# opendedup/sdfs

Hardware: AMD Instinct MI355X
Metric: device-resident GiB/s CDC+fingerprint, 4 KiB-mean chunks, 1/2/4/8 MI355X (higher is better)
Workload: dtype u8; 1 GPU; 64 streams x 64 MiB per GPU, CHUNK_LENGTH 262144 B (16384 buffers, 4.00 GiB per GPU), fresh CDC state per buffer; chunks_per_gpu_step=1059575, streams_in_flight=2, exchange=none (N=1), parallelism=dp1 (streams sharded per GPU)

## Files before the change

### sdfs_amd/csrc/cdc_device.h

```cpp
#pragma once

#include "cdc_internal.h"

namespace sdfs {

__device__ __forceinline__ uint32_t xor3(uint32_t a, uint32_t b, uint32_t c) {
    return __builtin_amdgcn_bitop3_b32(a, b, c, 0x96);
}
__device__ __forceinline__ uint32_t maj3(uint32_t a, uint32_t b, uint32_t c) {
    return __builtin_amdgcn_bitop3_b32(a, b, c, 0xE8);
}
__device__ __forceinline__ uint32_t bitop3_and_or(uint32_t a, uint32_t b, uint32_t c) {
    return __builtin_amdgcn_bitop3_b32(a, b, c, 0xEA);
}

constexpr int kAblMirror = 64;
constexpr int kAblSgprPred = 256;
constexpr int kAblFullBlocks = 512;

constexpr int kAblSdwa = 1024;
constexpr int kAblSdwaPop = 2048;
constexpr int kAblMinGroup = 4096;
constexpr int kAblMinGroup8 = 8192;
constexpr int kAblPopSwap = 16384;
constexpr int kAblPopMux = 32768;

template <int B>
__device__ __forceinline__ void sdwa_byte_to_b1(uint32_t& d, uint32_t src) {
    static_assert(B >= 0 && B < 4, "byte select");
    if constexpr (B == 0)
        asm("v_mov_b32_sdwa %0, %1 dst_sel:BYTE_1 dst_unused:UNUSED_PRESERVE src0_sel:BYTE_0" : "+v"(d) : "v"(src));
    else if constexpr (B == 1)
        asm("v_mov_b32_sdwa %0, %1 dst_sel:BYTE_1 dst_unused:UNUSED_PRESERVE src0_sel:BYTE_1" : "+v"(d) : "v"(src));
    else if constexpr (B == 2)
        asm("v_mov_b32_sdwa %0, %1 dst_sel:BYTE_1 dst_unused:UNUSED_PRESERVE src0_sel:BYTE_2" : "+v"(d) : "v"(src));
    else
        asm("v_mov_b32_sdwa %0, %1 dst_sel:BYTE_1 dst_unused:UNUSED_PRESERVE src0_sel:BYTE_3" : "+v"(d) : "v"(src));
}

template <int P, int Q, int ABL = 0>
__device__ __forceinline__ void roll_step(uint32_t& lo, uint32_t& hi, uint32_t dw, uint32_t odw, uint32_t& c8,
                                          uint32_t& push_base, uint32_t jshift, const uint8_t* tab) {
    if constexpr ((ABL & kAblMirror) != 0) {
        uint32_t pa, qa;
        if constexpr ((ABL & kAblSdwa) != 0) {
            asm("v_lshrrev_b32_sdwa %0, %2, %1 dst_sel:BYTE_1 dst_unused:UNUSED_PRESERVE src0_sel:DWORD src1_sel:DWORD"
                : "+v"(push_base)
                : "v"(lo), "s"(jshift));
            pa = push_base;
        } else {
            pa = bitop3_and_or(lo >> (jshift - 8), 0xFF00u, push_base);
        }
        if constexpr ((ABL & kAblSdwaPop) != 0 && (ABL & kAblPopMux) != 0 && Q == 2) {
            qa = __builtin_amdgcn_bitop3_b32(odw, 0xFF00u, c8, 0xE2);
        } else if constexpr ((ABL & kAblSdwaPop) != 0) {
            sdwa_byte_to_b1<3 - Q>(c8, odw);
            qa = c8;
        } else {
            qa = Q == 2 ? bitop3_and_or(odw, 0xFF00u, c8)
                        : __builtin_amdgcn_perm(odw, c8, 0x0C0C0000u | ((4u + 3 - Q) << 8));
        }
        const uint2 pv = (ABL & 2) ? make_uint2(pa, pa >> 3) : *reinterpret_cast<const uint2*>(tab + pa);
        const uint2 qv = (ABL & 1) ? make_uint2(qa, qa >> 3) : *reinterpret_cast<const uint2*>(tab + qa);
        const uint32_t nlo = __builtin_amdgcn_alignbit(hi, lo, 8);
        const uint32_t nhi = __builtin_amdgcn_perm(hi, dw, 0x00070605u | ((3u - P) << 24));
        if constexpr ((ABL & kAblPopSwap) != 0) {
            lo = xor3(nlo, pv.x, qv.y);
            hi = xor3(nhi, pv.y, qv.x);
        } else {
            lo = xor3(nlo, pv.x, qv.x);
            hi = xor3(nhi, pv.y, qv.y);
        }
        return;
    }
    const uint32_t pa = bitop3_and_or(hi >> (jshift - 8), 0xFF00u, push_base);
    const uint32_t qa = __builtin_amdgcn_perm(odw, c8, 0x0C0C0000u | ((4u + Q) << 8));
    const uint2 pv = (ABL & 2) ? make_uint2(pa, pa >> 3) : *reinterpret_cast<const uint2*>(tab + pa);
    const uint2 qv = (ABL & 1) ? make_uint2(qa, qa >> 3) : *reinterpret_cast<const uint2*>(tab + qa);
    const uint32_t nhi = __builtin_amdgcn_alignbit(hi, lo, 24);
    const uint32_t nlo = __builtin_amdgcn_perm(lo, dw, 0x06050400u | P);
    lo = xor3(nlo, pv.x, qv.x);
    hi = xor3(nhi, pv.y, qv.y);
}

template <int P, bool M = false>
__device__ __forceinline__ void push_step(uint32_t& lo, uint32_t& hi, uint32_t dw, uint32_t push_base,
                                          uint32_t jshift, const uint8_t* tab) {
    if constexpr (M) {
        const uint2 pv = *reinterpret_cast<const uint2*>(tab + bitop3_and_or(lo >> (jshift - 8), 0xFF00u, push_base));
        const uint32_t nlo = __builtin_amdgcn_alignbit(hi, lo, 8);
        const uint32_t nhi = __builtin_amdgcn_perm(hi, dw, 0x00070605u | ((3u - P) << 24));
        lo = nlo ^ pv.x;
        hi = nhi ^ pv.y;
        return;
    }
    const uint2 pv = *reinterpret_cast<const uint2*>(tab + bitop3_and_or(hi >> (jshift - 8), 0xFF00u, push_base));
    const uint32_t nhi = __builtin_amdgcn_alignbit(hi, lo, 24);
    const uint32_t nlo = __builtin_amdgcn_perm(lo, dw, 0x06050400u | P);
    lo = nlo ^ pv.x;
    hi = nhi ^ pv.y;
}

template <int PK>
__device__ __forceinline__ void cand_shift(uint32_t& bits, uint32_t lo, uint32_t hi, const ScanArgs& a) {
    if constexpr (PK == 3) {
        const uint32_t flo = __builtin_bitreverse32(lo), fhi = __builtin_bitreverse32(hi);
        const double f = __builtin_fma((double)fhi, 4294967296.0, (double)flo);
        const double q = __builtin_floor(f * a.div_inv);
        const double r = __builtin_fma(-q, a.div_d, f);
        const uint32_t h = (r == a.rem_d) | (r + a.div_d == a.rem_d) | (r - a.div_d == a.rem_d);
        asm("v_lshl_or_b32 %0, %0, 1, %1" : "+v"(bits) : "v"(h));
    } else if constexpr (PK == 2) {
        asm("v_cmp_gt_u32 vcc, %2, %1\n\t"
            "v_addc_co_u32 %0, vcc, %0, %0, vcc"
            : "+v"(bits)
            : "v"(lo), "s"(a.thr)
            : "vcc");
    } else if constexpr (PK == 1) {
        uint32_t t, t2;
        asm("v_and_b32 %1, %4, %3\n\t"
            "v_xor_b32 %1, %5, %1\n\t"
            "v_and_b32 %2, %7, %6\n\t"
            "v_xor_b32 %2, %8, %2\n\t"
            "v_or_b32 %1, %1, %2\n\t"
            "v_cmp_eq_u32 vcc, 0, %1\n\t"
            "v_addc_co_u32 %0, vcc, %0, %0, vcc"
            : "+v"(bits), "=&v"(t), "=&v"(t2)
            : "v"(lo), "s"(a.mask_lo), "s"(a.val_lo), "v"(hi), "s"(a.mask_hi), "s"(a.val_hi)
            : "vcc");
    } else {
        uint32_t t;
        asm("v_and_b32 %1, %3, %2\n\t"
            "v_cmp_eq_u32 vcc, %4, %1\n\t"
            "v_addc_co_u32 %0, vcc, %0, %0, vcc"
            : "+v"(bits), "=&v"(t)
            : "v"(lo), "s"(a.mask_lo), "s"(a.val_lo)
            : "vcc");
    }
}

template <int W, int PK, int O, int ABL, int BLKW>
__device__ __forceinline__ void byte_step(uint32_t& lo, uint32_t& hi, uint32_t& bits, const uint32_t (&cur)[BLKW],
                                          const uint32_t (&prev)[16], uint32_t& c8, uint32_t& push_base,
                                          const uint8_t* tab, const ScanArgs& a, uint64_t (&gm)[8], uint32_t (&hv)[8]) {
    constexpr int OLD = O - W;
    constexpr int OI = OLD >= 0 ? OLD : OLD + 64;
    const uint32_t odw = OLD >= 0 ? cur[OI >> 2] : prev[OI >> 2];
    roll_step<(O & 3), (OI & 3), ABL>(lo, hi, cur[O >> 2], odw, c8, push_base, a.jshift, tab);
    if constexpr ((ABL & 4) != 0 && (ABL & kAblSgprPred) != 0) {
        asm volatile("" ::"v"(hi));
    } else if constexpr (ABL & 4) {
        bits ^= lo;
    } else if constexpr ((ABL & kAblMinGroup) != 0 && (ABL & kAblMirror) != 0 && PK == 2) {
        constexpr int G = (ABL & kAblMinGroup8) != 0 ? 8 : 4;
        hv[O & (G - 1)] = hi;
        if constexpr ((O & (G - 1)) == G - 1) {
            uint32_t m = min(min(hv[0], hv[1]), hv[2]);
            m = min(m, hv[3]);
            if constexpr (G == 8) {
                m = min(min(m, hv[4]), hv[5]);
                m = min(min(m, hv[6]), hv[7]);
            }
            if (__builtin_expect(__any(m < a.thr), 0)) {
#pragma unroll
                for (int p = 0; p < G; p++) cand_shift<2>(bits, hv[p], 0u, a);
            } else {
                bits <<= G;
            }
        }
    } else if constexpr ((ABL & kAblSgprPred) != 0 && (ABL & kAblMirror) != 0 && PK == 2) {
        asm("v_cmp_gt_u32_e64 %0, %1, %2" : "=s"(gm[O & 7]) : "s"(a.thr), "v"(hi));
        if constexpr ((O & 7) == 7) {
            const uint64_t any = (gm[0] | gm[1]) | (gm[2] | gm[3]) | (gm[4] | gm[5]) | (gm[6] | gm[7]);
            if (__builtin_expect(any != 0, 0)) {
#pragma unroll
                for (int p = 0; p < 8; p++) {
                    uint64_t co;
                    asm volatile("v_addc_co_u32_e64 %0, %1, %0, %0, %2" : "+v"(bits), "=s"(co) : "s"(gm[p]));
// ... 448 lines not shown
                atomicOr(a.overflow, 1u);
            }
        }
        carry_rank += (uint32_t)__builtin_popcountll(cut[k]);
        const uint32_t mx = __builtin_amdgcn_readlane(wave_incl_max(end1), 63);
        carry_pos = mx > carry_pos ? mx : carry_pos;
    }
    if (lane == 0 && probe) {
        a.counts[b] = 0;
    } else if (lane == 0) {
        const uint32_t nchunks = cnt + (start < len ? 1u : 0u);
        if (start < len) {
            if (cnt < a.cap) {
                const uint64_t slot = (uint64_t)b * a.cap + cnt;
                a.starts[slot] = start;
                a.clens[slot] = len - start;
                uint32_t bin = sha_blocks(len - start) >> a.bin_shift;
                bin = bin < a.nbins ? bin : a.nbins - 1;
                atomicAdd(&lhist[bin], 1u);
            } else {
                atomicOr(a.overflow, 1u);
            }
        }
        a.counts[b] = nchunks < a.cap ? nchunks : a.cap;
    }
    return true;
}

__device__ __forceinline__ int64_t find_first_sum(const ResolveArgs& a, uint32_t b, uint32_t lo, uint32_t hi,
                                                  uint32_t lane) {
    const uint32_t sl = a.seg_len;
    const uint64_t spb = a.uniform_len / sl;
    const uint64_t word0 = ((uint64_t)b * a.uniform_len) >> 5;
    for (uint32_t s0 = lo / sl; s0 <= hi / sl; s0 += 64) {
        const uint32_t sj = s0 + lane;
        uint32_t best = 0xFFFFFFFFu;
        if (sj <= hi / sl) {
            const uint32_t* ss = a.seg_sum + ((uint64_t)b * spb + sj) * kSegSumWords;
            const uint4 q = *reinterpret_cast<const uint4*>(ss);
            const uint32_t nc = ss[4], ovf = ss[5];
            const uint32_t base = sj * sl;
            const uint32_t qw[4] = {q.x, q.y, q.z, q.w};
#pragma unroll
            for (int j = 0; j < 8; j++) {
                const uint32_t v = (qw[j >> 1] >> (16 * (j & 1))) & 0xFFFFu;
                const uint32_t c = base + v;
                if (v != 0xFFFFu && c >= lo && c <= hi && c < best) best = c;
            }
            if (best == 0xFFFFFFFFu && nc > kSumCands) {
                uint32_t x = base + ovf > lo ? base + ovf : lo;
                const uint32_t seg_hi = base + sl - 1;
                const uint32_t to = seg_hi < hi ? seg_hi : hi;
                while (x <= to) {
                    uint32_t w = a.bitmap[word0 + (x >> 5)] >> (x & 31);
                    const uint32_t span = to - x;
                    if (span < 31) w &= (2u << span) - 1u;
                    if (w) { best = x + __builtin_ctz(w); break; }
                    x = (x | 31u) + 1u;
                }
            }
        }
        const uint64_t m = __ballot(best != 0xFFFFFFFFu);
        if (m) return (int64_t)__builtin_amdgcn_readlane(best, (int)__builtin_ctzll(m));
    }
    return -1;
}

__device__ __forceinline__ void piece_walk_from_summary(const ResolveArgs& a, uint32_t item, uint32_t r0, uint32_t lane,
                                                        const uint32_t (&sm)[4], uint32_t ncand, uint32_t ovf_off,
                                                        uint32_t seg_len, uint64_t word0) {
    const uint32_t len = a.uniform_len;
    const uint32_t r1 = r0 + 64 * seg_len < len ? r0 + 64 * seg_len : len;
    const uint32_t my_base = r0 + lane * seg_len;
    uint32_t q0 = sm[0], q1 = sm[1], q2 = sm[2], q3 = sm[3];
    {
        const uint32_t sh = kSumCands - (ncand < kSumCands ? ncand : kSumCands);
        if (sh & 4) { q3 = q1; q2 = q0; q1 = 0xFFFFFFFFu; q0 = 0xFFFFFFFFu; }
        if (sh & 2) { q3 = q2; q2 = q1; q1 = q0; q0 = 0xFFFFFFFFu; }
        if (sh & 1) {
            q3 = __builtin_amdgcn_alignbit(q3, q2, 16);
            q2 = __builtin_amdgcn_alignbit(q2, q1, 16);
            q1 = __builtin_amdgcn_alignbit(q1, q0, 16);
            q0 = (q0 << 16) | 0xFFFFu;
        }
    }
    auto head_of = [&](uint32_t top) { return (top >> 16) == 0xFFFFu ? 0xFFFFFFFFu : my_base + (top >> 16); };
    uint32_t head = head_of(q3);
    const bool ovf = ncand > kSumCands;
    uint32_t* sp = a.spec_starts + (uint64_t)item * a.spec_cap;
    uint32_t start = r0, cnt = 0;
    while (start < r1) {
        if (lane == 0 && cnt < a.spec_cap) sp[cnt] = start;
        cnt++;
        const uint32_t lo = start + a.first_off;
        const uint32_t forced = start + a.max_len - 1;
        const uint32_t hi = forced < len - 1 ? forced : len - 1;
        const uint32_t hp = hi < r1 - 1 ? hi : r1 - 1;
        int64_t k = -1;
        if (lo <= hp) {
            for (;;) {
                const bool adv = head < lo;
                if (__ballot(adv) == 0) break;
                if (adv) {
                    q3 = __builtin_amdgcn_alignbit(q3, q2, 16);
                    q2 = __builtin_amdgcn_alignbit(q2, q1, 16);
                    q1 = __builtin_amdgcn_alignbit(q1, q0, 16);
                    q0 = (q0 << 16) | 0xFFFFu;
                    head = head_of(q3);
                }
            }
            uint32_t best = head <= hp ? head : 0xFFFFFFFFu;
            if (ovf && head == 0xFFFFFFFFu) {
                uint32_t x = my_base + ovf_off > lo ? my_base + ovf_off : lo;
                const uint32_t seg_hi = my_base + seg_len - 1;
                const uint32_t to = seg_hi < hp ? seg_hi : hp;
                while (x <= to) {
                    uint32_t w = a.bitmap[word0 + (x >> 5)] >> (x & 31);
                    const uint32_t span = to - x;
                    if (span < 31) w &= (2u << span) - 1u;
                    if (w) { best = x + __builtin_ctz(w); break; }
                    x = (x | 31u) + 1u;
                }
            }
            const uint64_t m = __ballot(best != 0xFFFFFFFFu);
            if (m) k = (int64_t)__builtin_amdgcn_readlane(best, (int)__builtin_ctzll(m));
        }
        if (k < 0) {
            if (hi > r1 - 1) break;
            k = (int64_t)hi;
        }
        start = (uint32_t)k + 1;
    }
    if (lane == 0) a.spec_cnt[item] = cnt < a.spec_cap ? cnt : a.spec_cap;
}

template <int C, int NCH, bool PF, int WPS, int ABL = 0, int BLK = 64, int FUSE = 0, int THREADS = kScanThreads,
          bool MIRROR = false>
struct ScanCfg {
    static constexpr bool kMirror = MIRROR;
    static constexpr bool kPopSwap = MIRROR && (ABL & kAblPopSwap) != 0;
    static constexpr int kFuse = NCH == 1 ? FUSE : (FUSE == 2 ? 2 : 0);
    static constexpr int kThreads = THREADS;
    static constexpr int kAbl = ABL;
    static constexpr int kCopies = C;
    static constexpr int kChains = NCH;
    static constexpr bool kPrefetch = PF;
    static constexpr int kWavesPerSimd = WPS;
    static constexpr int kLds = scan_lds_bytes(C);
    static constexpr uint32_t kPushOff = C == 32 ? 0x10000u : 0x80u;
    static constexpr int kBlk = BLK;
    static constexpr bool kListWalk = kFuse == 2 && NCH == 1 && C == 32;
};

template <int W, int PK, class CFG>
__device__ __forceinline__ void scan_iter(const ScanArgs& a, const uint8_t* tab, uint32_t* lhist, uint64_t base,
                                          uint32_t tid, uint32_t bdim, uint64_t total, uint32_t lane, uint32_t c8,
                                          uint32_t push_base, uint32_t& pa_reg, uint32_t& qa_reg,
                                          uint32_t* wlist = nullptr) {
    constexpr int MB =
        (CFG::kMirror ? kAblMirror : 0) | (CFG::kAbl & (kAblSgprPred | kAblSdwa | kAblSdwaPop | kAblMinGroup | kAblMinGroup8 | kAblPopSwap | kAblPopMux));
    constexpr int NCH = CFG::kChains;
    constexpr int BLK = CFG::kBlk;
    constexpr int BLKW = BLK / 4;
    uint64_t start[NCH], end[NCH];
    uint32_t nblk[NCH];
    bool first[NCH];
    uint32_t maxblk = 0;
#pragma unroll
    for (int c = 0; c < NCH; c++) {
        const uint64_t seg = base + (uint64_t)c * bdim + tid;
        start[c] = end[c] = 0;
        nblk[c] = 0;
        first[c] = true;
        if (seg < total) {
            uint64_t bstart, blen, sidx;
            if (a.uniform_len) {
                const uint64_t spb = (a.uniform_len + a.seg_len - 1) / a.seg_len;
                const uint64_t b = seg / spb;
                sidx = seg - b * spb;
                bstart = b * a.uniform_len;
                blen = a.uniform_len;
            } else {
                uint32_t lo_b = 0, hi_b = a.nbuf;
                while (hi_b - lo_b > 1) {
                    const uint32_t mid = (lo_b + hi_b) >> 1;
                    if (a.seg_prefix[mid] <= seg) lo_b = mid; else hi_b = mid;
                }
                sidx = seg - a.seg_prefix[lo_b];
                bstart = a.offs[lo_b];
                blen = a.lens[lo_b];
            }
            start[c] = bstart + sidx * a.seg_len;
            const uint64_t bend = bstart + blen;
            end[c] = start[c] + a.seg_len < bend ? start[c] + a.seg_len : bend;
            nblk[c] = (uint32_t)((end[c] - start[c] + BLK - 1) / BLK);
            first[c] = start[c] == bstart;
        }
        maxblk = nblk[c] > maxblk ? nblk[c] : maxblk;
    }

    uint32_t lo[NCH], hi[NCH];
    uint32_t prev[NCH][16], cur[NCH][BLKW];
    bool cur_full[NCH];
    uint32_t sm[NCH][4];
    uint32_t ncand[NCH];
    uint32_t ovf_off[NCH];
#pragma unroll
    for (int c = 0; c < NCH; c++) {
        sm[c][0] = sm[c][1] = sm[c][2] = sm[c][3] = 0xFFFFFFFFu;
        ncand[c] = 0;
        ovf_off[c] = 0xFFFFFFFFu;
    }
    const bool sparse_bm = CFG::kFuse == 2 && a.fuse_resolve != 0;
#pragma unroll
    for (int c = 0; c < NCH; c++) {
        if (nblk[c] != 0 && !first[c]) {
            load_block<16>(prev[c], a.data, start[c] - 64, start[c]);
            if constexpr (CFG::kMirror)
#pragma unroll
                for (int i = 0; i < 16; i++) prev[c][i] = __builtin_bitreverse32(prev[c][i]);
        } else {
#pragma unroll
            for (int i = 0; i < 16; i++) prev[c][i] = 0;
        }
        lo[c] = hi[c] = 0;
        warm_from<W, 64 - W, CFG::kMirror>(lo[c], hi[c], prev[c], push_base, a.jshift, tab);
        if constexpr (CFG::kPrefetch) {
            const bool act = nblk[c] != 0;
            cur_full[c] = load_block_nb<BLKW>(cur[c], a.data, a.zero_page, act ? start[c] : 0, act ? end[c] : 0);
        }
    }

    for (uint32_t blk = 0; blk < maxblk; blk++) {
        uint32_t nxt[NCH][CFG::kPrefetch ? BLKW : 1];
        bool nxt_full[NCH];
        uint32_t words[NCH][BLK / 32];
        bool split_fast = false;
        if constexpr ((CFG::kAbl & kAblFullBlocks) != 0) {
#pragma unroll
            for (int c = 0; c < NCH; c++) {
                const uint4* p = reinterpret_cast<const uint4*>(a.data + start[c] + (uint64_t)BLK * blk);
#pragma unroll
                for (int i = 0; i < BLKW / 4; i++) {
                    const uint4 v = p[i];
                    cur[c][4 * i] = v.x; cur[c][4 * i + 1] = v.y; cur[c][4 * i + 2] = v.z; cur[c][4 * i + 3] = v.w;
                }
            }
            block_words<W, PK, 0, BLK / 32, NCH, (CFG::kAbl & 7) | MB, BLKW>(words, lo, hi, cur, prev, qa_reg, pa_reg,
                                                                             tab, a);
            split_fast = true;
        } else if constexpr (CFG::kAbl & 16) {
            bool full = true;
#pragma unroll
            for (int c = 0; c < NCH; c++)
                full = full && blk < nblk[c] && start[c] + (uint64_t)BLK * (blk + 1) <= end[c];
            split_fast = __all(full);
            if (split_fast) {
#pragma unroll
                for (int c = 0; c < NCH; c++) {
                    const uint4* p = reinterpret_cast<const uint4*>(a.data + start[c] + (uint64_t)BLK * blk);
#pragma unroll
                    for (int i = 0; i < BLKW / 4; i++) {
                        const uint4 v = p[i];
                        cur[c][4 * i] = v.x; cur[c][4 * i + 1] = v.y; cur[c][4 * i + 2] = v.z; cur[c][4 * i + 3] = v.w;
                    }
                }
                block_words<W, PK, 0, BLK / 32, NCH, (CFG::kAbl & 3) | MB, BLKW>(words, lo, hi, cur, prev, qa_reg, pa_reg,
                                                                                 tab, a);
            }
        }
        if (!split_fast) {
#pragma unroll
        for (int c = 0; c < NCH; c++) {
            if constexpr (CFG::kPrefetch) {
                fix_block<BLKW>(cur[c], cur_full[c], a.data, start[c] + (uint64_t)BLK * blk, end[c]);
                const bool act = blk + 1 < nblk[c];
                nxt_full[c] = load_block_nb<BLKW>(nxt[c], a.data, a.zero_page,
                                                  act ? start[c] + (uint64_t)BLK * (blk + 1) : 0, act ? end[c] : 0);
            } else if constexpr (CFG::kAbl & 8) {
#pragma unroll
                for (int i = 0; i < BLKW; i++) cur[c][i] = prev[c][i & 15] * 0x9E3779B1u + blk;
            } else {
                const bool act = blk < nblk[c];
                load_block<BLKW>(cur[c], a.data, act ? start[c] + (uint64_t)BLK * blk : 0, act ? end[c] : 0);
            }
        }
        block_words<W, PK, 0, BLK / 32, NCH, (CFG::kAbl & 15) | MB, BLKW>(words, lo, hi, cur, prev, qa_reg, pa_reg, tab, a);
        }
        if constexpr (CFG::kFuse == 2) {
#pragma unroll
            for (int c = 0; c < NCH; c++)
#pragma unroll
                for (int w = 0; w < BLK / 32; w++) {
                    uint32_t bits = blk < nblk[c] ? words[c][w] : 0u;
                    while (bits) {
                        const uint32_t off = blk * BLK + 32 * w + __builtin_ctz(bits);
                        bits &= bits - 1;
                        if (start[c] + off < end[c]) sum_push(sm[c], ncand[c], off);
                    }
                }
        }
#pragma unroll
        for (int c = 0; c < NCH; c++) {
            if constexpr (CFG::kFuse == 2)
                if (ncand[c] > kSumCands && ovf_off[c] == 0xFFFFFFFFu) ovf_off[c] = blk * BLK;
            if (blk < nblk[c] && (!sparse_bm || ncand[c] > kSumCands)) {
                const uint64_t pos = start[c] + (uint64_t)BLK * blk;
                uint32_t* bm = a.bitmap + (pos >> 5);
                if (pos + BLK <= end[c]) {
                    if constexpr (BLK >= 128) {
#pragma unroll
                        for (int w = 0; w < BLK / 32; w += 4)
                            *reinterpret_cast<uint4*>(bm + w) =
                                make_uint4(words[c][w], words[c][w + 1], words[c][w + 2], words[c][w + 3]);
                    } else {
                        *reinterpret_cast<uint2*>(bm) = make_uint2(words[c][0], words[c][1]);
                    }
                } else {
#pragma unroll
                    for (int w = 0; w < BLK / 32; w++)
                        if (pos + 32 * w < end[c]) bm[w] = words[c][w];
                }
            }
#pragma unroll
            for (int i = 0; i < 16; i++) prev[c][i] = cur[c][BLKW - 16 + i];
            if constexpr (CFG::kPrefetch) {
#pragma unroll
                for (int i = 0; i < BLKW; i++) cur[c][i] = nxt[c][i];
                cur_full[c] = nxt_full[c];
            }
        }
    }
    if constexpr (CFG::kFuse != 0) {
        if (a.fuse_resolve && a.skip_walk != 1) {
            const uint64_t seg0 = base + (tid & ~63u);
            __builtin_amdgcn_fence(__ATOMIC_RELEASE, "workgroup");
            __builtin_amdgcn_fence(__ATOMIC_ACQUIRE, "workgroup");
            if constexpr (CFG::kFuse == 2) {
                if (a.fuse_resolve == 2) {
                    if constexpr (NCH == 1) {
                        if (base + tid < total) {
                            uint32_t* ss = a.res.seg_sum + (base + tid) * kSegSumWords;
                            *reinterpret_cast<uint4*>(ss) = make_uint4(sm[0][0], sm[0][1], sm[0][2], sm[0][3]);
                            *reinterpret_cast<uint2*>(ss + 4) = make_uint2(ncand[0], ovf_off[0]);
                        }
                        const uint64_t spb = a.uniform_len / a.seg_len;
                        const uint64_t b = seg0 / spb;
                        const uint32_t piece = (uint32_t)((seg0 - b * spb) >> 6);
                        if (seg0 < total)
                            piece_walk_from_summary(a.res, (uint32_t)b * a.res.nsec + piece, piece * 64 * a.seg_len,
                                                    lane, sm[0], ncand[0], ovf_off[0], a.seg_len,
                                                    (b * a.uniform_len) >> 5);
                    }
                } else {
#pragma unroll
                    for (int c = 0; c < NCH; c++) {
                        const uint64_t sc = seg0 + (uint64_t)c * bdim;
                        if (sc < total) {
                            bool done = false;
                            if constexpr (CFG::kListWalk)
                                if (wlist && a.list_walk)
                                    done = resolve_from_list(a.res, (uint32_t)(sc >> 6), lane, sm[c], ncand[c], a.seg_len,
                                                             lhist, wlist, a.skip_walk);
                            if (!done && a.skip_walk > 1) {
                                if (lane == 0) a.res.counts[(uint32_t)(sc >> 6)] = 0;
                            } else if (!done)
                                resolve_from_summary<(CFG::kAbl & 128) == 0>(a.res, (uint32_t)(sc >> 6), lane, sm[c],
                                                                             ncand[c], ovf_off[c], a.seg_len, lhist);
                        }
                    }
                }
            } else {
                if (seg0 < total) resolve_buffer(a.res, (uint32_t)(seg0 >> 6), lane, lhist);
            }
        }
    }
}

template <int W, int PK, class CFG>
__global__ __launch_bounds__(CFG::kThreads, CFG::kWavesPerSimd) void cdc_scan_kernel(ScanArgs a) {
    static_assert(!CFG::kMirror || !CFG::kPrefetch, "mirrored state: no prefetch");
    static_assert(CFG::kMirror || PK < 2, "the one-compare and divisor predicates need the mirrored state");
    constexpr int NCH = CFG::kChains;
    constexpr int C = CFG::kCopies;
    __shared__ __attribute__((aligned(16))) uint8_t tab[CFG::kLds];
    __shared__ uint32_t lhist[CFG::kFuse ? kMaxBins : 1];
    __shared__ uint32_t wlist[CFG::kListWalk ? CFG::kThreads / 64 * kListCap : 1];
    {
        const uint4* src = reinterpret_cast<const uint4*>(a.tab_image);
        uint4* dst = reinterpret_cast<uint4*>(tab);
        for (int i = threadIdx.x; i < CFG::kLds / 16; i += blockDim.x) dst[i] = src[i];
        if constexpr (CFG::kFuse != 0)
            for (uint32_t i = threadIdx.x; i < kMaxBins; i += blockDim.x) lhist[i] = 0;
    }
    __syncthreads();

    const uint32_t lane = threadIdx.x & 63;
    const uint32_t c8 = (lane & (C - 1)) << 3;
    const uint32_t push_base = CFG::kPushOff | c8;
    uint32_t pa_reg = push_base, qa_reg = c8;
    const uint64_t total = a.uniform_len ? a.total_segs : a.seg_prefix[a.nbuf];
    const uint64_t per_iter = (uint64_t)blockDim.x * NCH;

    uint32_t* const wl = CFG::kListWalk ? wlist + (threadIdx.x >> 6) * kListCap : nullptr;
    bool dyn = false;
    if constexpr (NCH == 1) dyn = a.wave_ctr != nullptr;
    const uint32_t items = (uint32_t)((total + 63) >> 6);
    uint64_t sbase = (uint64_t)blockIdx.x * per_iter;
    for (;;) {
        uint64_t base;
        uint32_t tid, bdim;
        if (dyn) {
            uint32_t it = 0;
            if (lane == 0) it = atomicAdd(a.wave_ctr, 1u);
            it = __builtin_amdgcn_readfirstlane(it);
            if (it >= items) break;
            base = (uint64_t)it * 64;
            tid = lane;
            bdim = 64;
        } else {
            if (sbase >= total) break;
            base = sbase;
            tid = threadIdx.x;
            bdim = blockDim.x;
            sbase += (uint64_t)gridDim.x * per_iter;
        }
        scan_iter<W, PK, CFG>(a, tab, lhist, base, tid, bdim, total, lane, c8, push_base, pa_reg, qa_reg, wl);
    }
    if constexpr (CFG::kFuse != 0) {
        if (a.fuse_resolve && a.skip_walk < 2) {
            __syncthreads();
            for (uint32_t i = threadIdx.x; i < a.res.nbins; i += blockDim.x)
                if (lhist[i]) atomicAdd(&a.res.hist[i], lhist[i]);
        }
    }
}

__device__ __forceinline__ uint32_t rotr(uint32_t x, uint32_t n) { return __builtin_amdgcn_alignbit(x, x, n); }

constexpr uint32_t kSha256K[64] = {
    0x428a2f98, 0x71374491, 0xb5c0fbcf, 0xe9b5dba5, 0x3956c25b, 0x59f111f1, 0x923f82a4, 0xab1c5ed5,
    0xd807aa98, 0x12835b01, 0x243185be, 0x550c7dc3, 0x72be5d74, 0x80deb1fe, 0x9bdc06a7, 0xc19bf174,
    0xe49b69c1, 0xefbe4786, 0x0fc19dc6, 0x240ca1cc, 0x2de92c6f, 0x4a7484aa, 0x5cb0a9dc, 0x76f988da,
    0x983e5152, 0xa831c66d, 0xb00327c8, 0xbf597fc7, 0xc6e00bf3, 0xd5a79147, 0x06ca6351, 0x14292967,
    0x27b70a85, 0x2e1b2138, 0x4d2c6dfc, 0x53380d13, 0x650a7354, 0x766a0abb, 0x81c2c92e, 0x92722c85,
    0xa2bfe8a1, 0xa81a664b, 0xc24b8b70, 0xc76c51a3, 0xd192e819, 0xd6990624, 0xf40e3585, 0x106aa070,
    0x19a4c116, 0x1e376c08, 0x2748774c, 0x34b0bcb5, 0x391c0cb3, 0x4ed8aa4a, 0x5b9cca4f, 0x682e6ff3,
    0x748f82ee, 0x78a5636f, 0x84c87814, 0x8cc70208, 0x90befffa, 0xa4506ceb, 0xbef9a3f7, 0xc67178f2};

template <bool SB = false>
__device__ __forceinline__ void sha256_compress(uint32_t (&s)[8], uint32_t (&w)[16]) {
    uint32_t a = s[0], b = s[1], c = s[2], d = s[3], e = s[4], f = s[5], g = s[6], h = s[7];
#pragma clang loop unroll(full)
    for (int i = 0; i < 64; i++) {
        if (i >= 16 && (i & 15) == 0) {
            asm("" : "+v"(w[0]), "+v"(w[1]), "+v"(w[2]), "+v"(w[3]), "+v"(w[4]), "+v"(w[5]), "+v"(w[6]),
                "+v"(w[7]), "+v"(w[8]), "+v"(w[9]), "+v"(w[10]), "+v"(w[11]), "+v"(w[12]), "+v"(w[13]),
                "+v"(w[14]), "+v"(w[15]) : "v"(a));
#pragma unroll
            for (int j = 0; j < 16; j++) {
                const uint32_t w15 = w[(j + 1) & 15], w2 = w[(j + 14) & 15];
                const uint32_t s0 = xor3(rotr(w15, 7), rotr(w15, 18), w15 >> 3);
                const uint32_t s1 = xor3(rotr(w2, 17), rotr(w2, 19), w2 >> 10);
                w[j] = w[j] + s0 + w[(j + 9) & 15] + s1;
            }
        }
        const uint32_t wi = w[i & 15];
        const uint32_t S1 = xor3(rotr(e, 6), rotr(e, 11), rotr(e, 25));
        const uint32_t ch = (e & f) | (~e & g);
        const uint32_t t1 = h + S1 + ch + kSha256K[i] + wi;
        const uint32_t S0 = xor3(rotr(a, 2), rotr(a, 13), rotr(a, 22));
        const uint32_t mj = maj3(a, b, c);
        h = g; g = f; f = e; e = d + t1; d = c; c = b; b = a; a = t1 + S0 + mj;
        if constexpr (SB) __builtin_amdgcn_sched_barrier(0);
    }
    s[0] += a; s[1] += b; s[2] += c; s[3] += d; s[4] += e; s[5] += f; s[6] += g; s[7] += h;
}

__device__ __forceinline__ uint32_t rotl(uint32_t x, uint32_t n) { return __builtin_amdgcn_alignbit(x, x, 32 - n); }

__device__ __forceinline__ void md5_compress(uint32_t (&s)[4], const uint32_t (&m)[16]) {
    constexpr uint32_t K[64] = {
        0xd76aa478, 0xe8c7b756, 0x242070db, 0xc1bdceee, 0xf57c0faf, 0x4787c62a, 0xa8304613, 0xfd469501,
        0x698098d8, 0x8b44f7af, 0xffff5bb1, 0x895cd7be, 0x6b901122, 0xfd987193, 0xa679438e, 0x49b40821,
        0xf61e2562, 0xc040b340, 0x265e5a51, 0xe9b6c7aa, 0xd62f105d, 0x02441453, 0xd8a1e681, 0xe7d3fbc8,
        0x21e1cde6, 0xc33707d6, 0xf4d50d87, 0x455a14ed, 0xa9e3e905, 0xfcefa3f8, 0x676f02d9, 0x8d2a4c8a,
        0xfffa3942, 0x8771f681, 0x6d9d6122, 0xfde5380c, 0xa4beea44, 0x4bdecfa9, 0xf6bb4b60, 0xbebfbc70,
        0x289b7ec6, 0xeaa127fa, 0xd4ef3085, 0x04881d05, 0xd9d4d039, 0xe6db99e5, 0x1fa27cf8, 0xc4ac5665,
        0xf4292244, 0x432aff97, 0xab9423a7, 0xfc93a039, 0x655b59c3, 0x8f0ccc92, 0xffeff47d, 0x85845dd1,
        0x6fa87e4f, 0xfe2ce6e0, 0xa3014314, 0x4e0811a1, 0xf7537e82, 0xbd3af235, 0x2ad7d2bb, 0xeb86d391};
    constexpr int R[16] = {7, 12, 17, 22, 5, 9, 14, 20, 4, 11, 16, 23, 6, 10, 15, 21};
    uint32_t a = s[0], b = s[1], c = s[2], d = s[3];
#pragma unroll
    for (int i = 0; i < 64; i++) {
        uint32_t f;
        int g;
        if (i < 16) { f = (b & c) | (~b & d); g = i; }
        else if (i < 32) { f = (d & b) | (~d & c); g = (5 * i + 1) & 15; }
        else if (i < 48) { f = xor3(b, c, d); g = (3 * i + 5) & 15; }
        else { f = c ^ (b | ~d); g = (7 * i) & 15; }
        const uint32_t t = a + f + K[i] + m[g];
        a = d; d = c; c = b;
        b = b + rotl(t, R[(i >> 4) * 4 + (i & 3)]);
    }
    s[0] += a; s[1] += b; s[2] += c; s[3] += d;
}

template <bool SHA>
__device__ __forceinline__ void tail_words(uint32_t (&m)[16], const uint8_t* t, uint32_t rem) {
    const uint32_t r = (uint32_t)(reinterpret_cast<uintptr_t>(t) & 3);
    const uint32_t* q = reinterpret_cast<const uint32_t*>(t - r);
    const uint32_t nd = (r + rem + 3) >> 2;
    uint32_t d[17];
#pragma unroll
    for (int j = 0; j < 17; j++) d[j] = (uint32_t)j < nd ? q[j] : 0u;
#pragma unroll
    for (int j = 0; j < 16; j++) {
        uint32_t v = __builtin_amdgcn_alignbyte(d[j + 1], d[j], r);
        const int k = (int)rem - 4 * j;
        if (k <= 0) v = 0;
        else if (k < 4) v &= (1u << (8 * k)) - 1u;
        if (k >= 0 && k < 4) v |= 0x80u << (8 * k);
        m[j] = SHA ? __builtin_bswap32(v) : v;
    }
}

__device__ __forceinline__ void load_block64(uint4 (&v)[4], const uint8_t* q) {
#pragma unroll
    for (int j = 0; j < 4; j++) __builtin_memcpy(&v[j], q + 16 * j, 16);
}

template <int ALGO>
__device__ __forceinline__ void store_digest(const HashArgs& a, uint32_t slot, uint32_t b, uint32_t k, uint32_t cs,
                                             uint32_t len, const uint32_t (&s)[8]) {
// ... 599 lines not shown
```

### sdfs_amd/csrc/cdc_kernels.hip

```cpp
#include <algorithm>

#include "cdc_device.h"

namespace sdfs {

using ScanProd = ScanCfg<32, 1, false, 4, 16 | kAblSdwa | kAblSdwaPop | kAblMinGroup | kAblMinGroup8 | kAblPopSwap, 256,
                         2, kScanThreads, true>;

using ScanTiny = ScanCfg<32, 1, false, 4, 16 | kAblSdwa | kAblSdwaPop | kAblMinGroup | kAblMinGroup8 | kAblPopSwap, 64,
                         0, kScanThreads, true>;

template <class CFG>
constexpr ScanVariantInfo info_of() {
    return {CFG::kCopies, CFG::kChains, CFG::kLds, std::max(1, CFG::kWavesPerSimd * 256 / CFG::kThreads), CFG::kBlk,
            CFG::kFuse, CFG::kThreads, CFG::kMirror, CFG::kPopSwap};
}

ScanVariantInfo scan_variant_info(int v) {
    if (v == 0) return info_of<ScanProd>();
#ifdef SDFS_TUNING
    return scan_variant_info_sweep(v);
#else
    return {0, 0, 0, 0, 0, 0, 0};
#endif
}

bool scan_window_supported(int window) {
    return window == 16 || window == 32 || window == 48 || window == 64;
}

template <int W, class CFG>
static hipError_t launch_scan_wc(const ScanArgs& a, int pk, int grid, int block, hipStream_t s) {
    static_assert(CFG::kMirror, "the production scan rolls the mirrored state");
    if (pk == 1)
        hipLaunchKernelGGL((cdc_scan_kernel<W, 1, CFG>), dim3(grid), dim3(block), 0, s, a);
    else if (pk == 2)
        hipLaunchKernelGGL((cdc_scan_kernel<W, 2, CFG>), dim3(grid), dim3(block), 0, s, a);
    else if (pk == 3)
        hipLaunchKernelGGL((cdc_scan_kernel<W, 3, CFG>), dim3(grid), dim3(block), 0, s, a);
    else
        hipLaunchKernelGGL((cdc_scan_kernel<W, 0, CFG>), dim3(grid), dim3(block), 0, s, a);
    return hipGetLastError();
}

hipError_t launch_scan(const ScanArgs& a, int window, int pk, int variant, int grid, int block, hipStream_t s) {
    if (variant != 0) {
#ifdef SDFS_TUNING
        return launch_scan_sweep(a, window, pk, variant, grid, block, s);
#else
        return hipErrorInvalidValue;
#endif
    }
    switch (window) {
    case 16: return launch_scan_wc<16, ScanProd>(a, pk, grid, block, s);
    case 32: return launch_scan_wc<32, ScanProd>(a, pk, grid, block, s);
    case 48: return launch_scan_wc<48, ScanProd>(a, pk, grid, block, s);
    case 64: return launch_scan_wc<64, ScanProd>(a, pk, grid, block, s);
    default: return hipErrorInvalidValue;
    }
}

hipError_t launch_scan_tiny(const ScanArgs& a, int window, int pk, int grid, int block, hipStream_t s) {
    if (a.fuse_resolve) return hipErrorInvalidValue;
    switch (window) {
    case 16: return launch_scan_wc<16, ScanTiny>(a, pk, grid, block, s);
    case 32: return launch_scan_wc<32, ScanTiny>(a, pk, grid, block, s);
    case 48: return launch_scan_wc<48, ScanTiny>(a, pk, grid, block, s);
    case 64: return launch_scan_wc<64, ScanTiny>(a, pk, grid, block, s);
    default: return hipErrorInvalidValue;
    }
}

__global__ __launch_bounds__(1024) void seg_prefix_kernel(const uint32_t* lens, uint32_t nbuf, uint32_t seg_len,
                                                          uint64_t* seg_prefix) {
    __shared__ uint64_t part[1024];
    const uint32_t t = threadIdx.x;
    const uint32_t per = (nbuf + 1023) / 1024;
    const uint32_t b0 = t * per, b1 = (b0 + per < nbuf) ? b0 + per : nbuf;
    uint64_t sum = 0;
    for (uint32_t b = b0; b < b1; b++) sum += (lens[b] + seg_len - 1) / seg_len;
    part[t] = sum;
    __syncthreads();
    for (uint32_t off = 1; off < 1024; off <<= 1) {
        const uint64_t v = t >= off ? part[t - off] : 0;
        __syncthreads();
        part[t] += v;
        __syncthreads();
    }
    uint64_t run = part[t] - sum;
    for (uint32_t b = b0; b < b1; b++) {
        seg_prefix[b] = run;
        run += (lens[b] + seg_len - 1) / seg_len;
    }
    if (t == 1023) seg_prefix[nbuf] = part[1023];
}

hipError_t launch_seg_prefix(const uint32_t* lens, uint32_t nbuf, uint32_t seg_len, uint64_t* seg_prefix,
                             hipStream_t s) {
    hipLaunchKernelGGL(seg_prefix_kernel, dim3(1), dim3(1024), 0, s, lens, nbuf, seg_len, seg_prefix);
    return hipGetLastError();
}

__global__ __launch_bounds__(256) void cdc_resolve_kernel(ResolveArgs a) {
    __shared__ uint32_t lhist[kMaxBins];
    for (uint32_t i = threadIdx.x; i < a.nbins; i += 256) lhist[i] = 0;
    __syncthreads();
    const uint32_t lane = threadIdx.x & 63;
    const uint32_t nw = gridDim.x * 4;
    for (uint32_t b = blockIdx.x * 4 + (threadIdx.x >> 6); b < a.nbuf; b += nw) resolve_buffer(a, b, lane, lhist);
    __syncthreads();
    for (uint32_t i = threadIdx.x; i < a.nbins; i += 256)
        if (lhist[i]) atomicAdd(&a.hist[i], lhist[i]);
}

constexpr uint32_t kResStride = 6144;
constexpr uint32_t kResWin = 2 * kResStride;
constexpr uint32_t kResStage = kResWin / 2 / 192;

__device__ __forceinline__ int64_t find_first_lds(const uint32_t* win, uint32_t wbase, uint32_t lo_w, uint32_t lo_b,
                                                  uint32_t hi_w, uint32_t hi_b, uint32_t lane) {
    for (uint32_t wb = lo_w; wb <= hi_w; wb += 512) {
        const uint32_t w0 = wb + 8 * lane;
        uint32_t bits[8];
        uint32_t any = 0;
#pragma unroll
        for (int j = 0; j < 8; j++) {
            const uint32_t w = w0 + j;
            uint32_t v = 0;
            if (w <= hi_w) {
                v = win[w - wbase];
                if (w == lo_w) v &= ~0u << lo_b;
                if (w == hi_w) v &= hi_b == 31 ? ~0u : ((2u << hi_b) - 1u);
            }
            bits[j] = v;
            any |= v;
        }
        const uint64_t m = __ballot(any != 0);
        if (m) {
            const uint32_t l = __builtin_ctzll(m);
            uint32_t jj = 0, bb = 0;
#pragma unroll
            for (int j = 7; j >= 0; j--)
                if (bits[j]) { jj = j; bb = bits[j]; }
            const uint32_t pos_in = jj * 32 + (bb ? __builtin_ctz(bb) : 0);
            const uint32_t p = __shfl(pos_in, l);
            return (int64_t)(wb + 8 * l) * 32 + p;
        }
    }
    return -1;
}

__device__ __forceinline__ void stage_window(uint32_t* slot, const uint32_t* bm, uint64_t word0, uint64_t wbase,
                                             uint64_t nwords, uint32_t t, uint32_t nthreads_div) {
    const uint2* src = reinterpret_cast<const uint2*>(bm + word0 + wbase);
    uint2* dst = reinterpret_cast<uint2*>(slot);
    const uint64_t avail = nwords > wbase ? nwords - wbase : 0;
    uint2 v[kResStage];
#pragma unroll
    for (uint32_t k = 0; k < kResStage; k++) {
        const uint32_t i = t + k * nthreads_div;
// ... 887 lines not shown
```

### sdfs_amd/csrc/cdc_sweep_r3.hip

```cpp
#include <algorithm>

#include "cdc_device.h"

namespace sdfs {

using ScanV43 = ScanCfg<32, 1, false, 4, 16 | kAblSgprPred | kAblSdwa, 256, 2, kScanThreads, true>;
using ScanV44 = ScanCfg<32, 1, false, 4, 16 | kAblSgprPred | kAblSdwa | kAblSdwaPop, 256, 2, kScanThreads, true>;
using ScanV45 = ScanCfg<32, 1, false, 4, 16 | kAblSgprPred | kAblSdwa | kAblFullBlocks, 256, 2, kScanThreads, true>;
using ScanV46 = ScanCfg<16, 1, false, 6, 16 | kAblSgprPred | kAblSdwa, 128, 2, 768, true>;
using ScanV47 = ScanCfg<16, 1, false, 5, 16 | kAblSgprPred | kAblSdwa, 128, 2, 640, true>;
constexpr int kProdR3 = 16 | kAblSdwa | kAblSdwaPop;
using ScanV48 = ScanCfg<32, 1, false, 4, kProdR3 | kAblMinGroup, 256, 2, kScanThreads, true>;
using ScanV49 = ScanCfg<32, 1, false, 4, kProdR3 | kAblMinGroup | kAblMinGroup8, 256, 2, kScanThreads, true>;
using ScanV50 = ScanCfg<32, 1, false, 4, kProdR3 | kAblSgprPred | kAblPopSwap, 256, 2, kScanThreads, true>;
using ScanV51 = ScanCfg<32, 1, false, 4, kProdR3 | kAblMinGroup | kAblMinGroup8 | kAblPopSwap, 256, 2, kScanThreads, true>;
using ScanV52 = ScanCfg<32, 1, false, 4, kProdR3 | kAblMinGroup | kAblMinGroup8 | kAblPopSwap | kAblPopMux, 256, 2,
                        kScanThreads, true>;
using ScanV53 = ScanCfg<32, 1, false, 4, kProdR3 | kAblSgprPred | kAblPopSwap | kAblPopMux, 256, 2, kScanThreads, true>;

template <class CFG>
constexpr ScanVariantInfo info_r3() {
    return {CFG::kCopies, CFG::kChains, CFG::kLds, std::max(1, CFG::kWavesPerSimd * 256 / CFG::kThreads), CFG::kBlk,
            CFG::kFuse, CFG::kThreads, CFG::kMirror, CFG::kPopSwap};
}

ScanVariantInfo scan_variant_info_sweep_r3(int v) {
    switch (v) {
    case 43: return info_r3<ScanV43>();
    case 44: return info_r3<ScanV44>();
    case 45: return info_r3<ScanV45>();
    case 46: return info_r3<ScanV46>();
    case 47: return info_r3<ScanV47>();
    case 48: return info_r3<ScanV48>();
    case 49: return info_r3<ScanV49>();
    case 50: return info_r3<ScanV50>();
    case 51: return info_r3<ScanV51>();
    case 52: return info_r3<ScanV52>();
    case 53: return info_r3<ScanV53>();
    default: return {0, 0, 0, 0, 0, 0, 0, 0};
    }
}

template <class T>
static hipError_t launch_r3(const ScanArgs& a, int pk, int grid, int block, hipStream_t s) {
    static_assert(T::kMirror, "round-3 variants are mirrored-state forms");
    if ((T::kAbl & kAblFullBlocks) != 0 && !scan_full_blocks(a, T::kBlk)) return hipErrorInvalidValue;
    if (pk != 2) return hipErrorInvalidValue;
    hipLaunchKernelGGL((cdc_scan_kernel<48, 2, T>), dim3(grid), dim3(block), 0, s, a);
    return hipGetLastError();
}

hipError_t launch_scan_sweep_r3(const ScanArgs& a, int window, int pk, int variant, int grid, int block,
                                hipStream_t s) {
    if (window != 48) return hipErrorInvalidValue;
    switch (variant) {
    case 43: return launch_r3<ScanV43>(a, pk, grid, block, s);
    case 44: return launch_r3<ScanV44>(a, pk, grid, block, s);
    case 45: return launch_r3<ScanV45>(a, pk, grid, block, s);
    case 46: return launch_r3<ScanV46>(a, pk, grid, block, s);
    case 47: return launch_r3<ScanV47>(a, pk, grid, block, s);
    case 48: return launch_r3<ScanV48>(a, pk, grid, block, s);
    case 49: return launch_r3<ScanV49>(a, pk, grid, block, s);
    case 50: return launch_r3<ScanV50>(a, pk, grid, block, s);
    case 51: return launch_r3<ScanV51>(a, pk, grid, block, s);
    case 52: return launch_r3<ScanV52>(a, pk, grid, block, s);
    case 53: return launch_r3<ScanV53>(a, pk, grid, block, s);
    default: return hipErrorInvalidValue;
    }
}

template <int NS, int SP = 0>
static void fused_launch(const ScanArgs& a, const HashArgs& ha, uint32_t* ctr, int grid, hipStream_t s) {
    using Prod = ScanV51;
    if (ha.algo == 2)
        hipLaunchKernelGGL((cdc_fused_kernel<48, 2, Prod, 2, NS, SP>), dim3(grid), dim3(1024), 0, s, a, ha, ctr);
    else
        hipLaunchKernelGGL((cdc_fused_kernel<48, 2, Prod, 0, NS, SP>), dim3(grid), dim3(1024), 0, s, a, ha, ctr);
}

hipError_t launch_fused_probe(const ScanArgs& a, const HashArgs& ha, uint32_t* ctr, int window, int pk, int grid,
                              int form, hipStream_t s) {
    if (window != 48 || pk != 2 || !a.uniform_len || !a.fuse_resolve) return hipErrorInvalidValue;
    switch (form) {
    case 1: fused_launch<0>(a, ha, ctr, grid, s); break;
    case 2: fused_launch<1>(a, ha, ctr, grid, s); break;
    case 3: fused_launch<2>(a, ha, ctr, grid, s); break;
    case 4: fused_launch<3>(a, ha, ctr, grid, s); break;
    case 5: fused_launch<1, 2>(a, ha, ctr, grid, s); break;
    case 6: fused_launch<0, 2>(a, ha, ctr, grid, s); break;
    case 7: fused_launch<3, 2>(a, ha, ctr, grid, s); break;
    default: return hipErrorInvalidValue;
    }
    return hipGetLastError();
}

}
```

Measured before the change: 1058 GiB/s.

## Add two-half register ring prefetch to the production CDC scan loop

```diff
diff --git a/sdfs_amd/csrc/cdc_device.h b/sdfs_amd/csrc/cdc_device.h
--- a/sdfs_amd/csrc/cdc_device.h
+++ b/sdfs_amd/csrc/cdc_device.h
@@ -24,6 +24,8 @@
 constexpr int kAblMinGroup8 = 8192;
 constexpr int kAblPopSwap = 16384;
 constexpr int kAblPopMux = 32768;
+constexpr int kAblRing = 65536;
+constexpr int kAblNoLoadXor = 131072;
 
 template <int B>
 __device__ __forceinline__ void sdwa_byte_to_b1(uint32_t& d, uint32_t src) {
@@ -778,6 +780,35 @@
     static constexpr bool kListWalk = kFuse == 2 && NCH == 1 && C == 32;
 };
 
+template <class CFG>
+__device__ __forceinline__ void ring_half_out(const ScanArgs& a, const uint32_t (&w)[1][4], uint64_t start,
+                                              uint64_t end, uint32_t off0, bool act, bool sparse_bm,
+                                              uint32_t (&sm)[4], uint32_t& ncand, uint32_t& ovf_off) {
+    if constexpr (CFG::kFuse == 2) {
+#pragma unroll
+        for (int k = 0; k < 4; k++) {
+            uint32_t bits = act ? w[0][k] : 0u;
+            while (bits) {
+                const uint32_t off = off0 + 32 * k + __builtin_ctz(bits);
+                bits &= bits - 1;
+                if (start + off < end) sum_push(sm, ncand, off);
+            }
+        }
+        if (ncand > kSumCands && ovf_off == 0xFFFFFFFFu) ovf_off = off0;
+    }
+    if (act && (!sparse_bm || ncand > kSumCands)) {
+        const uint64_t pos = start + off0;
+        uint32_t* bm = a.bitmap + (pos >> 5);
+        if (pos + 128 <= end) {
+            *reinterpret_cast<uint4*>(bm) = make_uint4(w[0][0], w[0][1], w[0][2], w[0][3]);
+        } else {
+#pragma unroll
+            for (int k = 0; k < 4; k++)
+                if (pos + 32 * k < end) bm[k] = w[0][k];
+        }
+    }
+}
+
 template <int W, int PK, class CFG>
 __device__ __forceinline__ void scan_iter(const ScanArgs& a, const uint8_t* tab, uint32_t* lhist, uint64_t base,
                                           uint32_t tid, uint32_t bdim, uint64_t total, uint32_t lane, uint32_t c8,
@@ -827,6 +858,10 @@
 
     uint32_t lo[NCH], hi[NCH];
     uint32_t prev[NCH][16], cur[NCH][BLKW];
+    constexpr bool kRing = (CFG::kAbl & kAblRing) != 0;
+    static_assert(!kRing || (NCH == 1 && BLK == 256 && !CFG::kPrefetch),
+                  "the ring is the one-chain 256-byte block loop's own prefetch");
+    uint32_t rx[NCH][kRing ? 32 : 1], ry[NCH][kRing ? 32 : 1];
     bool cur_full[NCH];
     uint32_t sm[NCH][4];
     uint32_t ncand[NCH];
@@ -850,6 +885,10 @@
             for (int i = 0; i < 16; i++) prev[c][i] = 0;
         }
         lo[c] = hi[c] = 0;
+        if constexpr (kRing) {
+            load_block_nb<32>(rx[c], a.data, a.zero_page, start[c], end[c]);
+            load_block_nb<32>(ry[c], a.data, a.zero_page, start[c] + 128, end[c]);
+        }
         warm_from<W, 64 - W, CFG::kMirror>(lo[c], hi[c], prev[c], push_base, a.jshift, tab);
         if constexpr (CFG::kPrefetch) {
             const bool act = nblk[c] != 0;
@@ -857,6 +896,37 @@
         }
     }
 
+    if constexpr (kRing) {
+        constexpr int RA = (CFG::kAbl & 3) | MB;
+        const uint32_t seg_bytes = (uint32_t)(end[0] - start[0]);
+        const bool act = nblk[0] != 0;
+        const uint32_t nh = (seg_bytes + 127) / 128;
+        const uint32_t nh_max = __builtin_amdgcn_readlane(wave_incl_max(nh), 63);
+        const uint32_t whole = act ? seg_bytes / BLK : 0xFFFFFFFFu;
+        uint32_t nring = ~__builtin_amdgcn_readlane(wave_incl_max(~whole), 63);
+        nring = nring < nh_max / 2 ? nring : nh_max / 2;
+        uint32_t w4[1][4];
+        for (uint32_t blk = 0; blk < nring; blk++) {
+            block_words<W, PK, 0, 4, 1, RA, 32>(w4, lo, hi, rx, prev, qa_reg, pa_reg, tab, a);
+            ring_half_out<CFG>(a, w4, start[0], end[0], blk * BLK, act, sparse_bm, sm[0], ncand[0], ovf_off[0]);
+#pragma unroll
+            for (int i = 0; i < 16; i++) prev[0][i] = rx[0][16 + i];
+            load_block_nb<32>(rx[0], a.data, a.zero_page, start[0] + (uint64_t)BLK * (blk + 1), end[0]);
+            block_words<W, PK, 0, 4, 1, RA, 32>(w4, lo, hi, ry, prev, qa_reg, pa_reg, tab, a);
+            ring_half_out<CFG>(a, w4, start[0], end[0], blk * BLK + 128, act, sparse_bm, sm[0], ncand[0], ovf_off[0]);
+#pragma unroll
+            for (int i = 0; i < 16; i++) prev[0][i] = ry[0][16 + i];
+            load_block_nb<32>(ry[0], a.data, a.zero_page, start[0] + (uint64_t)BLK * (blk + 1) + 128, end[0]);
+        }
+        for (uint32_t h = 2 * nring; h < nh_max; h++) {
+            const bool ah = h < nh;
+            load_block<32>(rx[0], a.data, ah ? start[0] + 128ull * h : 0, ah ? end[0] : 0);
+            block_words<W, PK, 0, 4, 1, RA, 32>(w4, lo, hi, rx, prev, qa_reg, pa_reg, tab, a);
+            ring_half_out<CFG>(a, w4, start[0], end[0], h * 128, ah, sparse_bm, sm[0], ncand[0], ovf_off[0]);
+#pragma unroll
+            for (int i = 0; i < 16; i++) prev[0][i] = rx[0][16 + i];
+        }
+    } else
     for (uint32_t blk = 0; blk < maxblk; blk++) {
         uint32_t nxt[NCH][CFG::kPrefetch ? BLKW : 1];
         bool nxt_full[NCH];
@@ -903,6 +973,9 @@
                 const bool act = blk + 1 < nblk[c];
                 nxt_full[c] = load_block_nb<BLKW>(nxt[c], a.data, a.zero_page,
                                                   act ? start[c] + (uint64_t)BLK * (blk + 1) : 0, act ? end[c] : 0);
+            } else if constexpr ((CFG::kAbl & 8) != 0 && (CFG::kAbl & kAblNoLoadXor) != 0) {
+#pragma unroll
+                for (int i = 0; i < BLKW; i++) cur[c][i] = prev[c][i & 15] ^ (blk + (uint32_t)(i >> 4));
             } else if constexpr (CFG::kAbl & 8) {
 #pragma unroll
                 for (int i = 0; i < BLKW; i++) cur[c][i] = prev[c][i & 15] * 0x9E3779B1u + blk;
@@ -1005,7 +1078,6 @@
 
 template <int W, int PK, class CFG>
 __global__ __launch_bounds__(CFG::kThreads, CFG::kWavesPerSimd) void cdc_scan_kernel(ScanArgs a) {
-    static_assert(!CFG::kMirror || !CFG::kPrefetch, "mirrored state: no prefetch");
     static_assert(CFG::kMirror || PK < 2, "the one-compare and divisor predicates need the mirrored state");
     constexpr int NCH = CFG::kChains;
     constexpr int C = CFG::kCopies;
diff --git a/sdfs_amd/csrc/cdc_kernels.hip b/sdfs_amd/csrc/cdc_kernels.hip
--- a/sdfs_amd/csrc/cdc_kernels.hip
+++ b/sdfs_amd/csrc/cdc_kernels.hip
@@ -4,8 +4,9 @@
 
 namespace sdfs {
 
-using ScanProd = ScanCfg<32, 1, false, 4, 16 | kAblSdwa | kAblSdwaPop | kAblMinGroup | kAblMinGroup8 | kAblPopSwap, 256,
-                         2, kScanThreads, true>;
+using ScanProd = ScanCfg<32, 1, false, 4,
+                         16 | kAblSdwa | kAblSdwaPop | kAblMinGroup | kAblMinGroup8 | kAblPopSwap | kAblRing, 256, 2,
+                         kScanThreads, true>;
 
 using ScanTiny = ScanCfg<32, 1, false, 4, 16 | kAblSdwa | kAblSdwaPop | kAblMinGroup | kAblMinGroup8 | kAblPopSwap, 64,
                          0, kScanThreads, true>;
diff --git a/sdfs_amd/csrc/cdc_sweep_r3.hip b/sdfs_amd/csrc/cdc_sweep_r3.hip
--- a/sdfs_amd/csrc/cdc_sweep_r3.hip
+++ b/sdfs_amd/csrc/cdc_sweep_r3.hip
@@ -17,6 +17,9 @@
 using ScanV52 = ScanCfg<32, 1, false, 4, kProdR3 | kAblMinGroup | kAblMinGroup8 | kAblPopSwap | kAblPopMux, 256, 2,
                         kScanThreads, true>;
 using ScanV53 = ScanCfg<32, 1, false, 4, kProdR3 | kAblSgprPred | kAblPopSwap | kAblPopMux, 256, 2, kScanThreads, true>;
+using ScanV54 = ScanCfg<32, 1, false, 4, kAblSgprPred | 8 | kAblNoLoadXor, 256, 2, kScanThreads, true>;
+using ScanV55 = ScanCfg<32, 1, false, 4, kProdR3 | kAblMinGroup | kAblMinGroup8 | kAblPopSwap | kAblRing, 256, 2,
+                        kScanThreads, true>;
 
 template <class CFG>
 constexpr ScanVariantInfo info_r3() {
@@ -37,6 +40,8 @@
     case 51: return info_r3<ScanV51>();
     case 52: return info_r3<ScanV52>();
     case 53: return info_r3<ScanV53>();
+    case 54: return info_r3<ScanV54>();
+    case 55: return info_r3<ScanV55>();
     default: return {0, 0, 0, 0, 0, 0, 0, 0};
     }
 }
@@ -65,6 +70,8 @@
     case 51: return launch_r3<ScanV51>(a, pk, grid, block, s);
     case 52: return launch_r3<ScanV52>(a, pk, grid, block, s);
     case 53: return launch_r3<ScanV53>(a, pk, grid, block, s);
+    case 54: return launch_r3<ScanV54>(a, pk, grid, block, s);
+    case 55: return launch_r3<ScanV55>(a, pk, grid, block, s);
     default: return hipErrorInvalidValue;
     }
 }
```

Result: no change. 1071 GiB/s (median of 4 runs) (+1.2%).
